# NYXFLOWER/GripNet

Measured on NVIDIA B200. Metric: GripNet fwd+bwd edges/sec per epoch (pose-0 shape), higher is better.
Workload: dtype f32

## Files before the change

gripnet_b200/csrc/gemm.cu:

```cuda
#include "common.cuh"

namespace gn {

constexpr int kBK = 16;
constexpr int kGemmThreads = 256;
constexpr int kTargetCtas = 148 * 2;
constexpr int kMaxSplits = 3 * 148;

struct GemmParams {
  int M, N, K;
  const float* A; int64_t lda;
  const float* B; int64_t ldb;
  float* C; int64_t ldc;
  int batch; int64_t sA, sB, sC;
  int batch_reduce;
  float alpha; int accumulate;
  const float* addend; int64_t ldd;
  const float* mask; int64_t ldm;
  const int64_t* a_rows;
  int kt;
  int iters;
  int splits;
  int iters_per_split;
  int vec_ok;
  float* ws;
};

struct GemmPlan {
  int cfg;
  int bm, bn, bk;
  int splits, iters_per_split, iters, kt;
  int batch_indep;
};

static GemmPlan make_plan(int M, int N, int K, int batch, int batch_reduce, int allow_split) {
  GemmPlan pl;
  if (M >= 1024) {
    if (N <= 16) { pl.cfg = 2; pl.bm = 128; pl.bn = 16; }
    else if (N <= 32) { pl.cfg = 1; pl.bm = 128; pl.bn = 32; }
    else { pl.cfg = 0; pl.bm = 64; pl.bn = 64; }
  } else if (M <= 32 || N <= 32 || int64_t(M) * N <= 4096 * 4) {
    pl.cfg = 3; pl.bm = 32; pl.bn = 32;
  } else {
    pl.cfg = 0; pl.bm = 64; pl.bn = 64;
  }
  pl.bk = kBK;
  if (pl.cfg == 3 && K >= 256) { pl.cfg = 4; pl.bk = 64; }
  pl.kt = int(ceil_div(K, pl.bk));
  pl.batch_indep = batch_reduce ? 1 : batch;
  pl.iters = (batch_reduce ? batch : 1) * pl.kt;
  const int64_t tiles = ceil_div(M, pl.bm) * ceil_div(N, pl.bn) * pl.batch_indep;
  int splits = 1;
  if (allow_split && pl.iters >= 4 && tiles < kTargetCtas) {
    int64_t want = (pl.bk >= 64 ? 3 * 148 : kTargetCtas) / tiles;
    int64_t cap = pl.bk >= 64 ? pl.iters : pl.iters / 2;
    splits = int(want < cap ? want : cap);
    if (splits > kMaxSplits) splits = kMaxSplits;
    if (splits < 1) splits = 1;
  }
  pl.iters_per_split = int(ceil_div(pl.iters > 0 ? pl.iters : 1, splits));
  pl.splits = int(ceil_div(pl.iters > 0 ? pl.iters : 1, pl.iters_per_split));
  return pl;
}

template <int TN>
__device__ __forceinline__ void epilogue_row(const GemmParams& p, float* C, int m, int n0, const float (&v)[TN]) {
  float r[TN];
#pragma unroll
  for (int j = 0; j < TN; ++j) r[j] = v[j] * p.alpha;
  float* crow = C + int64_t(m) * p.ldc + n0;
  if (TN == 4 && p.vec_ok && n0 + 3 < p.N) {
    if (p.accumulate) {
      const float4 c = *reinterpret_cast<const float4*>(crow);
      r[0] += c.x; r[1] += c.y; r[2] += c.z; r[3] += c.w;
    }
    if (p.addend) {
      const float4 a = *reinterpret_cast<const float4*>(p.addend + int64_t(m) * p.ldd + n0);
      r[0] += a.x; r[1] += a.y; r[2] += a.z; r[3] += a.w;
    }
    if (p.mask) {
      const float4 k = *reinterpret_cast<const float4*>(p.mask + int64_t(m) * p.ldm + n0);
      if (!(k.x > 0.f)) r[0] = 0.f;
      if (!(k.y > 0.f)) r[1] = 0.f;
      if (!(k.z > 0.f)) r[2] = 0.f;
      if (!(k.w > 0.f)) r[3] = 0.f;
    }
    *reinterpret_cast<float4*>(crow) = make_float4(r[0], r[1], r[2], r[3]);
    return;
  }
#pragma unroll
  for (int j = 0; j < TN; ++j) {
    const int n = n0 + j;
    if (n >= p.N) break;
    float x = r[j];
    if (p.accumulate) x += crow[j];
    if (p.addend) x += p.addend[int64_t(m) * p.ldd + n];
    if (p.mask && !(p.mask[int64_t(m) * p.ldm + n] > 0.f)) x = 0.f;
    crow[j] = x;
  }
}

template <bool TA, bool TB, int BM, int BN, int TM, int TN, int BK>
__global__ void __launch_bounds__(kGemmThreads) sgemm_kernel(const GemmParams p) {
  constexpr int NTX = BN / TN;
  static_assert((BM / TM) * NTX == kGemmThreads, "tile / micro-tile mismatch");
  __shared__ __align__(16) float As[BK][BM + 4];
  __shared__ __align__(16) float Bs[BK][BN + 4];
  const int tid = threadIdx.x;
  const int tx = tid % NTX, ty = tid / NTX;
  const int m0 = blockIdx.x * BM, n0 = blockIdx.y * BN;
  const int zb = blockIdx.z / p.splits;
  const int zs = blockIdx.z - zb * p.splits;

  const int it_begin = zs * p.iters_per_split;
  const int it_end = min(p.iters, it_begin + p.iters_per_split);

  float acc[TM][TN];
#pragma unroll
  for (int i = 0; i < TM; ++i)
#pragma unroll
    for (int j = 0; j < TN; ++j) acc[i][j] = 0.f;

  for (int it = it_begin; it < it_end; ++it) {
    int b, k0;
    if (p.batch_reduce) { b = it / p.kt; k0 = (it - b * p.kt) * BK; } else { b = zb; k0 = it * BK; }
    const float* A = p.A + int64_t(b) * p.sA;
    const float* B = p.B + int64_t(b) * p.sB;
#pragma unroll
    for (int i = 0; i < (BM * BK) / kGemmThreads; ++i) {
      const int e = tid + i * kGemmThreads;
      int m, k;
      if (!TA) { k = e % BK; m = e / BK; } else { m = e % BM; k = e / BM; }
      const int gm = m0 + m, gk = k0 + k;
      float v = 0.f;
      if (gm < p.M && gk < p.K) {
        if (!TA) {
          const int64_t r = p.a_rows ? p.a_rows[gm] : gm;
          v = __ldg(A + r * p.lda + gk);
        } else {
          const int64_t r = p.a_rows ? p.a_rows[gk] : gk;
          v = __ldg(A + r * p.lda + gm);
        }
      }
      As[k][m] = v;
    }
#pragma unroll
    for (int i = 0; i < (BN * BK) / kGemmThreads; ++i) {
      const int e = tid + i * kGemmThreads;
      int n, k;
      if (!TB) { n = e % BN; k = e / BN; } else { k = e % BK; n = e / BK; }
      const int gn_ = n0 + n, gk = k0 + k;
      float v = 0.f;
      if (gn_ < p.N && gk < p.K) v = !TB ? __ldg(B + int64_t(gk) * p.ldb + gn_) : __ldg(B + int64_t(gn_) * p.ldb + gk);
      Bs[k][n] = v;
    }
    __syncthreads();
#pragma unroll
    for (int k = 0; k < BK; ++k) {
      float a[TM], bb[TN];
#pragma unroll
      for (int i = 0; i < TM; ++i) a[i] = As[k][ty * TM + i];
#pragma unroll
      for (int j = 0; j < TN; ++j) bb[j] = Bs[k][tx * TN + j];
#pragma unroll
      for (int i = 0; i < TM; ++i)
#pragma unroll
        for (int j = 0; j < TN; ++j) acc[i][j] = fmaf(a[i], bb[j], acc[i][j]);
    }
    __syncthreads();
  }

  if (p.splits > 1) {
    float* W = p.ws + (int64_t(zb) * p.splits + zs) * p.M * p.N;
#pragma unroll
    for (int i = 0; i < TM; ++i) {
      const int m = m0 + ty * TM + i;
      if (m >= p.M) continue;
#pragma unroll
      for (int j = 0; j < TN; ++j) {
        const int n = n0 + tx * TN + j;
        if (n < p.N) W[int64_t(m) * p.N + n] = acc[i][j];
      }
    }
    return;
  }
  float* C = p.C + (p.batch_reduce ? 0 : int64_t(zb) * p.sC);
#pragma unroll
  for (int i = 0; i < TM; ++i) {
    const int m = m0 + ty * TM + i;
    if (m < p.M) epilogue_row<TN>(p, C, m, n0 + tx * TN, acc[i]);
  }
}

template <int LANES>
__global__ void __launch_bounds__(256) splitk_reduce_kernel(const GemmParams p, int batch_indep) {
  const int64_t t = int64_t(blockIdx.x) * blockDim.x + threadIdx.x;
  const int64_t idx = t / LANES;
  const int lane = int(t % LANES);
  const int64_t mn = int64_t(p.M) * p.N;
  if (idx >= mn * batch_indep) return;
  const int zb = int(idx / mn);
  const int64_t o = idx - int64_t(zb) * mn;
  const float* w = p.ws + int64_t(zb) * p.splits * mn + o;
  float s = 0.f;
  int z = lane;
  for (; z + 3 * LANES < p.splits; z += 4 * LANES) {
    const float a = __ldcg(w + int64_t(z) * mn), b = __ldcg(w + int64_t(z + LANES) * mn);
    const float c = __ldcg(w + int64_t(z + 2 * LANES) * mn), d = __ldcg(w + int64_t(z + 3 * LANES) * mn);
    s += a; s += b; s += c; s += d;
  }
  for (; z < p.splits; z += LANES) s += __ldcg(w + int64_t(z) * mn);
  if (LANES == 32) {
#pragma unroll
    for (int off = 16; off > 0; off >>= 1) s += __shfl_xor_sync(kFull, s, off);
    if (lane != 0) return;
  }
  const float v[1] = {s};
  epilogue_row<1>(p, p.C + (p.batch_reduce ? 0 : int64_t(zb) * p.sC), int(o / p.N), int(o % p.N), v);
}

template <bool TA, bool TB>
static int launch_cfg(const GemmPlan& pl, const GemmParams& p, dim3 grid, cudaStream_t st) {
  switch (pl.cfg) {
    case 0: GN_LAUNCH((sgemm_kernel<TA, TB, 64, 64, 4, 4, 16>), grid, kGemmThreads, 0, st, p); break;
    case 1: GN_LAUNCH((sgemm_kernel<TA, TB, 128, 32, 4, 4, 16>), grid, kGemmThreads, 0, st, p); break;
    case 2: GN_LAUNCH((sgemm_kernel<TA, TB, 128, 16, 2, 4, 16>), grid, kGemmThreads, 0, st, p); break;
    case 3: GN_LAUNCH((sgemm_kernel<TA, TB, 32, 32, 2, 2, 16>), grid, kGemmThreads, 0, st, p); break;
    default: GN_LAUNCH((sgemm_kernel<TA, TB, 32, 32, 2, 2, 64>), grid, kGemmThreads, 0, st, p); break;
  }
  return GN_OK;
}

}

using namespace gn;

extern "C" size_t gn_sgemm_workspace_bytes(int32_t M, int32_t N, int32_t K, int32_t batch, int batch_reduce) {
  if (M <= 0 || N <= 0 || K <= 0 || batch < 1) return 0;
  const GemmPlan pl = make_plan(M, N, K, batch, batch_reduce, 1);
  if (pl.splits <= 1) return 0;
  return size_t(pl.batch_indep) * pl.splits * M * N * sizeof(float);
}

extern "C" int gn_sgemm(int transA, int transB, int32_t M, int32_t N, int32_t K, const float* A, int64_t lda,
                        const float* B, int64_t ldb, float* C, int64_t ldc, int32_t batch, int64_t strideA,
                        int64_t strideB, int64_t strideC, int batch_reduce, float alpha, int accumulate,
                        const float* addend, int64_t ld_addend, const float* relu_mask, int64_t ld_mask,
                        const int64_t* a_rows, int32_t split_k, float* ws, size_t ws_bytes, void* stream) {
  if (M < 0 || N < 0 || K < 0 || batch < 1 || !C) return GN_ERR_ARG;
  if (M == 0 || N == 0) return GN_OK;
  if (K > 0 && (!A || !B)) return GN_ERR_ARG;
  cudaStream_t st = as_stream(stream);
  const GemmPlan pl = make_plan(M, N, K, batch, batch_reduce, split_k > 0 && ws != nullptr);
  GemmParams p;
  p.M = M; p.N = N; p.K = K;
  p.A = A; p.lda = lda; p.B = B; p.ldb = ldb; p.C = C; p.ldc = ldc;
  p.batch = batch; p.sA = strideA; p.sB = strideB; p.sC = strideC;
  p.batch_reduce = batch_reduce ? 1 : 0;
  p.alpha = alpha; p.accumulate = accumulate ? 1 : 0;
  p.addend = addend; p.ldd = ld_addend; p.mask = relu_mask; p.ldm = ld_mask;
  p.a_rows = a_rows;
  p.kt = pl.kt; p.iters = pl.iters; p.splits = pl.splits; p.iters_per_split = pl.iters_per_split;
  p.ws = ws;
  auto al16 = [](const void* q) { return (reinterpret_cast<uintptr_t>(q) & 15u) == 0; };
  p.vec_ok = al16(C) && ldc % 4 == 0 && (batch_reduce || batch == 1 || strideC % 4 == 0) &&
             (!addend || (al16(addend) && ld_addend % 4 == 0)) && (!relu_mask || (al16(relu_mask) && ld_mask % 4 == 0));
  if (pl.splits > 1 && ws_bytes < size_t(pl.batch_indep) * pl.splits * M * N * sizeof(float)) return GN_ERR_WORKSPACE;
  const int64_t gz = int64_t(pl.batch_indep) * pl.splits;
  dim3 grid((unsigned)ceil_div(M, pl.bm), (unsigned)ceil_div(N, pl.bn), (unsigned)gz);
  if (grid.y > 65535 || gz > 65535) return GN_ERR_RANGE;
  if (!transA && !transB) GN_CHECK((launch_cfg<false, false>(pl, p, grid, st)));
  else if (!transA && transB) GN_CHECK((launch_cfg<false, true>(pl, p, grid, st)));
  else if (transA && !transB) GN_CHECK((launch_cfg<true, false>(pl, p, grid, st)));
  else GN_CHECK((launch_cfg<true, true>(pl, p, grid, st)));
  if (pl.splits > 1) {
    const int64_t total = int64_t(M) * N * pl.batch_indep;
    if (pl.splits >= 16 && total <= 8192) {
      GN_LAUNCH(splitk_reduce_kernel<32>, (unsigned)ceil_div(total * 32, 256), 256, 0, st, p, pl.batch_indep);
    } else {
      GN_LAUNCH(splitk_reduce_kernel<1>, (unsigned)ceil_div(total, 256), 256, 0, st, p, pl.batch_indep);
    }
  }
  return GN_OK;
}
```

gripnet_b200/ops.py:

```python
import os
import weakref

import torch

from . import _lib, streams
from .graph import _ptr, _stream, _ws, require_cuda, validate_index

EPS = 1e-13


class M:
    __slots__ = ("t", "ptr", "ld", "n", "f")

    def __init__(self, t, col0=0, width=None):
        assert t.dim() == 2 and t.stride(1) == 1 and t.dtype == torch.float32
        self.t = t
        self.n = t.size(0)
        self.f = t.size(1) - col0 if width is None else width
        self.ld = t.stride(0) if t.size(0) > 1 else max(t.size(1), 1)
        self.ptr = t.data_ptr() + 4 * col0


def _as_rows(x, name):
    require_cuda(x, name)
    if x.dtype != torch.float32:
        raise RuntimeError(f"gripnet_b200: {name} must be float32")
    if x.dim() != 2:
        raise RuntimeError(f"gripnet_b200: {name} must be 2-D")
    if x.stride(1) != 1 or (x.size(0) > 1 and x.stride(0) < x.size(1)):
        x = x.contiguous()
    return x


def _new(n, f, like):
    return torch.empty((n, f), dtype=torch.float32, device=like.device)


class Slot:
    __slots__ = ("m", "full", "dctx", "halo")

    def __init__(self, n_local, f, like, dctx=None, block=None, halo=None):
        self.dctx, self.halo = dctx, halo
        if dctx is None:
            t = _new(n_local, f, like)
            self.m, self.full = M(t), M(t)
        elif halo is not None:
            buf = dctx.slot_buffer(halo.rows, f, like, uniform=False)
            self.full = M(buf)
            self.m = M(buf[:n_local])
        else:
            buf = dctx.slot_buffer(dctx.world * block, f, like)
            self.full = M(buf)
            self.m = M(buf[dctx.rank * block: dctx.rank * block + n_local])

    def gather(self):
        if self.dctx is not None:
            if self.halo is not None:
                self.dctx.halo_gather(self.full.t, self.halo)
            else:
                self.dctx.all_gather_slots(self.full.t)
        return self.full


def _reduce(dctx, t):
    if dctx is not None:
        dctx.reduce_param_grad_(t)
    return t


def spmm(csr, x, out, F, row_scale=None, bias=None, addend=None, relu=False):
    lib = _lib.load()
    partial = csr.partial(min(F, 128))
    _lib.check(lib.gn_spmm(csr.ref, x.ptr, x.ld, F, _ptr(row_scale), _ptr(bias),
                           addend.ptr if addend is not None else None, addend.ld if addend is not None else 0,
                           int(relu), out.ptr, out.ld, _ptr(partial), _stream()), "gn_spmm")


GEMM_PATH = os.environ.get("GRIPNET_B200_GEMM", "auto")
_TC_MIN_M = 4096


def _tc_eligible(ta, m, n, k, a_ptr, lda, c_ptr, ldc, batch, alpha, accumulate, addend, mask, a_rows):
    if GEMM_PATH == "ffma" or ta or batch != 1 or a_rows is not None or accumulate or alpha != 1.0:
        return False
    if GEMM_PATH != "tc" and (m < _TC_MIN_M or k < 16):
        return False
    if k % 4 or lda % 4 or ldc % 4 or a_ptr % 16 or c_ptr % 16 or k > 4096:
        return False
    for e in (addend, mask):
        if e is not None and (e.ld % 4 or e.ptr % 16):
            return False
    return True


def sgemm(ta, tb, m, n, k, a_ptr, lda, b_ptr, ldb, c_ptr, ldc, device, batch=1, sa=0, sb=0, sc=0, batch_reduce=False,
          alpha=1.0, accumulate=False, addend=None, mask=None, a_rows=None, split_k=True):
    lib = _lib.load()
    if m > 0 and n > 0 and k > 0 and _tc_eligible(ta, m, n, k, a_ptr, lda, c_ptr, ldc, batch, alpha, accumulate,
                                                  addend, mask, a_rows):
        nbytes = int(lib.gn_tc_gemm_workspace_bytes(m, n, k))
        if nbytes:
            img = _ws(nbytes, device)
            _lib.check(lib.gn_tc_gemm(int(tb), m, n, k, a_ptr, lda, b_ptr, ldb, c_ptr, ldc,
                                      addend.ptr if addend is not None else None,
                                      addend.ld if addend is not None else 0,
                                      mask.ptr if mask is not None else None, mask.ld if mask is not None else 0,
                                      _ptr(img), nbytes, _stream()), "gn_tc_gemm")
            return
    ws, ws_bytes = None, 0
    if split_k:
        ws_bytes = int(lib.gn_sgemm_workspace_bytes(m, n, k, batch, int(batch_reduce)))
        if ws_bytes:
            ws = torch.empty(ws_bytes // 4, dtype=torch.float32, device=device)
            streams.keep(ws)
    _lib.check(lib.gn_sgemm(int(ta), int(tb), m, n, k, a_ptr, lda, b_ptr, ldb, c_ptr, ldc, batch, sa, sb, sc,
                            int(batch_reduce), float(alpha), int(accumulate),
                            addend.ptr if addend is not None else None, addend.ld if addend is not None else 0,
                            mask.ptr if mask is not None else None, mask.ld if mask is not None else 0,
                            _ptr(a_rows), 1 if ws is not None else 0, _ptr(ws), ws_bytes, _stream()), "gn_sgemm")


def _rel_tc_ok(k, ldx, ldy, x_ptr, y_ptr):
    return GEMM_PATH != "ffma" and k % 4 == 0 and ldx % 4 == 0 and ldy % 4 == 0 and x_ptr % 16 == 0 and y_ptr % 16 == 0


def rel_transform(x, w, y, r, k, f, device, image=None):
    lib = _lib.load()
    n = x.n
    if n == 0:
        return
    if _rel_tc_ok(k, x.ld, y.ld, x.ptr, y.ptr):
        if image is not None:
            _lib.check(lib.gn_tc_gemm_rel_image(n, r, f, k, x.ptr, x.ld, _ptr(image), image.numel(), y.ptr, y.ld,
                                                _stream()), "gn_tc_gemm_rel_image")
            return
        nbytes = int(lib.gn_tc_gemm_rel_workspace_bytes(n, r, f, k))
        if nbytes:
            img = _ws(nbytes, device)
            _lib.check(lib.gn_tc_gemm_rel(n, r, f, k, x.ptr, x.ld, w.data_ptr(), y.ptr, y.ld, _ptr(img), nbytes,
                                          _stream()), "gn_tc_gemm_rel")
            return
    sgemm(False, False, n, f, k, x.ptr, x.ld, w.data_ptr(), f, y.ptr, y.ld, device, batch=r, sa=0, sb=k * f, sc=f)


def rel_weights(basis, att):
    nb, k, f = basis.shape
    r = att.size(0)
    bs, at = basis.contiguous(), att.contiguous()
    w = torch.empty((r, k, f), dtype=torch.float32, device=basis.device)
    sgemm(False, False, r, k * f, nb, at.data_ptr(), nb, bs.data_ptr(), k * f, w.data_ptr(), k * f, basis.device)
    return w


class RelPrologue:

    _pending = {}

    def __init__(self, layers, n_rows):
        lib = _lib.load()
        self.branch = streams.Branch(background=True)
        self.entries = []
        flat = [t for pair in layers for t in pair]
        with self.branch(*flat):
            for basis, att in layers:
                w = rel_weights(basis.detach(), att.detach())
                nb, k, f = basis.shape
                r = att.size(0)
                image = None
                nbytes = int(lib.gn_tc_gemm_rel_workspace_bytes(n_rows, r, f, k)) if GEMM_PATH != "ffma" and k % 4 == 0 else 0
                if nbytes and n_rows > 0:
                    image = _ws(nbytes, basis.device)
                    _lib.check(lib.gn_tc_rel_image(n_rows, r, f, k, w.data_ptr(), _ptr(image), nbytes, _stream()),
                               "gn_tc_rel_image")
                key = (basis.data_ptr(), att.data_ptr())
                entry = (self.branch, basis._version, att._version, int(n_rows), w, image)
                RelPrologue._pending.pop(key, None)
                RelPrologue._pending[key] = entry
                self.entries.append(key)
        while len(RelPrologue._pending) > 16:
            RelPrologue._pending.pop(next(iter(RelPrologue._pending)))

    @staticmethod
    def take(basis, att, n_rows):
        e = RelPrologue._pending.pop((basis.data_ptr(), att.data_ptr()), None)
        if e is None:
            return None
        branch, vb, va, rows, w, image = e
        branch.join()
        if vb != basis._version or va != att._version:
            return None
        return w, (image if rows == int(n_rows) else None)


_TC_TN_MIN_ROWS = 1 << 15


def weight_grad(a, b, out, device, c_inner=0, c_stride=0, force_tc=False):
    lib = _lib.load()
    n, mo, no = a.n, a.f, b.f
    ok = GEMM_PATH != "ffma" and n > 0 and mo % 4 == 0 and no % 4 == 0 and a.ld % 4 == 0 and b.ld % 4 == 0 and \
        a.ptr % 16 == 0 and b.ptr % 16 == 0 and (force_tc or GEMM_PATH == "tc" or n >= _TC_TN_MIN_ROWS)
    if not ok:
        return False
    nbytes = int(lib.gn_tc_tn_workspace_bytes(n, mo, no))
    if not nbytes:
        return False
    ws = _ws(nbytes, device)
    _lib.check(lib.gn_tc_tn(a.ptr, a.ld, b.ptr, b.ld, n, mo, no, out.data_ptr(), no, int(c_inner), int(c_stride),
                            _ptr(ws), nbytes, _stream()), "gn_tc_tn")
    return True


def map2d(op, src, dst):
    _lib.check(_lib.load().gn_map2d(op, src.ptr, src.ld, dst.ptr, dst.ld, src.n, src.f, _stream()), "gn_map2d")


def relu_bwd(g, y, dst):
    _lib.check(_lib.load().gn_relu_bwd(g.ptr, g.ld, y.ptr, y.ld, dst.ptr, dst.ld, g.n, g.f, _stream()), "gn_relu_bwd")


def colsum(x, out):
    lib = _lib.load()
    ws = _ws(lib.gn_colsum_workspace_bytes(x.n, x.f), out.device)
    _lib.check(lib.gn_colsum(x.ptr, x.ld, x.n, x.f, _ptr(out), _ptr(ws), ws.numel(), _stream()), "gn_colsum")


class GcnStack(torch.autograd.Function):
    @staticmethod
    def forward(ctx, x0, graph, relu_flags, catout, *params):
        n_layers = len(relu_flags)
        weights = [params[2 * l] for l in range(n_layers)]
        biases = [params[2 * l + 1] for l in range(n_layers)]
        x0 = _as_rows(x0, "x")
        if x0.size(0) != graph.n_src:
            raise RuntimeError(f"x has {x0.size(0)} rows but the graph has {graph.n_src} source nodes")
        if catout and graph.n_src != graph.n_dst:
            raise RuntimeError("if_catout needs a square graph")
        dims = [x0.size(1)] + [w.size(1) for w in weights]
        for l, w in enumerate(weights):
            require_cuda(w, "weight", torch.float32)
            if w.size(0) != dims[l]:
                raise RuntimeError(f"layer {l}: weight expects {w.size(0)} input features, got {dims[l]}")
        dev = x0.device
        dctx = getattr(graph, "ctx", None)
        b_src = graph.b_src if dctx is not None else None
        outs = []
        br = streams.Branch()
        if catout:
            buf = _new(graph.n_dst, sum(dims), x0)
            offs = [sum(dims[:i]) for i in range(len(dims))]
            h0 = M(buf, offs[0], dims[0])
            outs.append(h0)
        else:
            buf = None
            outs.append(M(x0))
        for l in range(n_layers):
            w = weights[l].contiguous()
            k, f = dims[l], dims[l + 1]
            y = Slot(graph.n_src, f, x0, dctx, b_src, getattr(graph, "fwd_halo", None))
            xin = M(x0) if l == 0 else outs[l]
            sgemm(False, False, graph.n_src, f, k, xin.ptr, xin.ld, w.data_ptr(), f, y.m.ptr, y.m.ld, dev)
            if l == 0 and catout:
                with br(x0):
                    map2d(_lib.EW_COPY, M(x0), h0)
            if catout:
                hl = M(buf, offs[l + 1], f)
            else:
                hl = M(_new(graph.n_dst, f, x0))
            b = biases[l].contiguous() if biases[l] is not None else None
            spmm(graph.fwd, y.gather(), hl, f, bias=b, relu=relu_flags[l])
            outs.append(hl)
        br.join()
        ctx.graph, ctx.relu_flags, ctx.catout, ctx.dims = graph, relu_flags, catout, dims
        ctx.has_bias = [b is not None for b in biases]
        ctx.param_refs = [None if p is None else weakref.ref(p) for p in params]
        ws = [w.contiguous() for w in weights]
        acts = [buf] if catout else [o.t for o in outs]
        ctx.n_acts = len(acts)
        ctx.save_for_backward(*acts, *ws)
        return buf if catout else outs[-1].t

    @staticmethod
    def backward(ctx, grad_out):
        graph, relu_flags, catout, dims = ctx.graph, ctx.relu_flags, ctx.catout, ctx.dims
        n_layers = len(relu_flags)
        saved = ctx.saved_tensors
        acts, weights = saved[: ctx.n_acts], saved[ctx.n_acts:]
        if catout:
            offs0 = [sum(dims[:i]) for i in range(len(dims))]
            outs = [M(acts[0], offs0[i], dims[i]) for i in range(len(dims))]
        else:
            outs = [M(a) for a in acts]
        g = _as_rows(grad_out, "grad")
        dev = g.device
        dctx = getattr(graph, "ctx", None)
        b_dst = graph.b_dst if dctx is not None else None
        bwd_halo = getattr(graph, "bwd_halo", None)
        if catout:
            offs = [sum(dims[:i]) for i in range(len(dims))]
            gs = [M(g, offs[i], dims[i]) for i in range(len(dims))]
            dh = gs[n_layers]
        else:
            gs = None
            dh = M(g)
        grads = [None] * (2 * n_layers)
        dz_slot = None
        dx0 = None
        br = streams.Branch(enabled=dctx is None or dctx.defer_grad_reduce, background=True)
        br_b = streams.Branch(enabled=dctx is None or dctx.defer_grad_reduce, background=True)
        for l in range(n_layers, 0, -1):
            f, k = dims[l], dims[l - 1]
            h_l, h_prev = outs[l], outs[l - 1]
            if dz_slot is not None:
                dz = dz_slot
            elif relu_flags[l - 1]:
                dz = Slot(graph.n_dst, f, g, dctx, b_dst, bwd_halo)
                relu_bwd(dh, h_l, dz.m)
            elif dctx is not None:
                dz = Slot(graph.n_dst, f, g, dctx, b_dst, bwd_halo)
                map2d(_lib.EW_COPY, dh, dz.m)
            else:
                dz = Slot.__new__(Slot)
                dz.m, dz.full, dz.dctx = dh, dh, None
            if ctx.has_bias[l - 1] and ctx.needs_input_grad[4 + 2 * (l - 1) + 1]:
                db = torch.empty(f, dtype=torch.float32, device=dev)
                with br_b(dz.m.t):
                    colsum(dz.m, db)
                grads[2 * (l - 1) + 1] = _reduce(dctx, db)
            dy = M(_new(graph.n_src, f, g))
            spmm(graph.bwd, dz.gather(), dy, f)
            if ctx.needs_input_grad[4 + 2 * (l - 1)]:
                dw = torch.empty((k, f), dtype=torch.float32, device=dev)
                with br(dy.t, h_prev.t):
                    if not weight_grad(h_prev, dy, dw, dev):
                        sgemm(True, False, k, f, graph.n_src, h_prev.ptr, h_prev.ld, dy.ptr, dy.ld, dw.data_ptr(),
                              f, dev)
                grads[2 * (l - 1)] = _reduce(dctx, dw)
            need_prev = (l > 1) or ctx.needs_input_grad[0]
            dz_slot = None
            if need_prev:
                w = weights[l - 1]
                addend = gs[l - 1] if catout else None
                mask = h_prev if (l > 1 and relu_flags[l - 2]) else None
                dprev = Slot(graph.n_src, k, g, dctx if mask is not None else None, b_dst, bwd_halo)
                sgemm(False, True, graph.n_src, k, f, dy.ptr, dy.ld, w.data_ptr(), f, dprev.m.ptr, dprev.m.ld, dev,
                      addend=addend, mask=mask)
                dh = dprev.m
                if mask is not None:
                    dz_slot = dprev
                if l == 1:
                    dx0 = dprev.m.t
        defer = _only_stored(ctx, dctx)
        br_b.join(deferrable=defer)
        br.join(deferrable=defer)
        return (dx0, None, None, None) + tuple(grads)


def _only_stored(ctx, dctx):
    if dctx is not None and not dctx.defer_grad_reduce:
        return False
    params = [None if r is None else r() for r in ctx.param_refs]
    return streams.grads_only_stored(params, ctx.needs_input_grad[4:])


class RgcnStack(torch.autograd.Function):
    @staticmethod
    def forward(ctx, x0, graph, relu_flags, catout, *params):
        n_layers = len(relu_flags)
        basis = [params[4 * l] for l in range(n_layers)]
        att = [params[4 * l + 1] for l in range(n_layers)]
        root = [params[4 * l + 2] for l in range(n_layers)]
        bias = [params[4 * l + 3] for l in range(n_layers)]
        x0 = _as_rows(x0, "x")
        n, r = graph.n_nodes, graph.n_rel
        if x0.size(0) != n:
            raise RuntimeError(f"x has {x0.size(0)} rows but the graph has {n} nodes")
        dims = [x0.size(1)] + [rt.size(1) for rt in root]
        dev = x0.device
        dctx = getattr(graph, "ctx", None)
        blk = graph.b if dctx is not None else None
        outs, ws_list = [], []
        br = streams.Branch()
        if catout:
            buf = _new(n, sum(dims), x0)
            offs = [sum(dims[:i]) for i in range(len(dims))]
            h0 = M(buf, offs[0], dims[0])
            with br(x0):
                map2d(_lib.EW_COPY, M(x0), h0)
            outs.append(h0)
        else:
            buf = None
            outs.append(M(x0))
        for l in range(n_layers):
            k, f = dims[l], dims[l + 1]
            nb = basis[l].size(0)
            if att[l].size(0) != r:
                raise RuntimeError("att rows must equal the number of relations of the graph")
            bs, at, rt = basis[l].contiguous(), att[l].contiguous(), root[l].contiguous()
            n_in = n if dctx is None else dctx.world * blk
            pre = RelPrologue.take(basis[l], att[l], n_in)
            w, image = pre if pre is not None else (rel_weights(bs, at), None)
            xin = M(x0) if l == 0 else outs[l]
            hl = M(buf, offs[l + 1], f) if catout else M(_new(n, f, x0))
            with br(xin.t, rt, hl.t):
                sgemm(False, False, n, f, k, xin.ptr, xin.ld, rt.data_ptr(), f, hl.ptr, hl.ld, dev)
            if dctx is not None:
                xs = Slot(n, k, x0, dctx, blk)
                map2d(_lib.EW_COPY, xin, xs.m)
                xall = xs.gather()
            else:
                xall = xin
            yfull = _new(xall.n, r * f, x0)
            rel_transform(xall, w, M(yfull), r, k, f, dev, image=image if xall.n == n_in else None)
            b = bias[l].contiguous() if bias[l] is not None else None
            br.join()
            spmm(graph.fwd, M(yfull.view(yfull.size(0) * r, f)), hl, f, row_scale=graph.inv_cnt, bias=b, addend=hl,
                 relu=relu_flags[l])
            outs.append(hl)
            ws_list.append((w, bs, at, rt))
        br.join()
        ctx.graph, ctx.relu_flags, ctx.catout, ctx.dims = graph, relu_flags, catout, dims
        ctx.has_bias = [b is not None for b in bias]
        ctx.param_refs = [None if p is None else weakref.ref(p) for p in params]
        acts = [buf] if catout else [o.t for o in outs]
        ctx.n_acts = len(acts)
        flat = [t for tup in ws_list for t in tup]
        ctx.save_for_backward(*acts, *flat)
        return buf if catout else outs[-1].t

    @staticmethod
    def backward(ctx, grad_out):
        graph, relu_flags, catout, dims = ctx.graph, ctx.relu_flags, ctx.catout, ctx.dims
        n_layers = len(relu_flags)
        n, r = graph.n_nodes, graph.n_rel
        saved = ctx.saved_tensors
        acts, flat = saved[: ctx.n_acts], saved[ctx.n_acts:]
        ws_list = [tuple(flat[4 * i: 4 * i + 4]) for i in range(n_layers)]
        if catout:
            offs0 = [sum(dims[:i]) for i in range(len(dims))]
            outs = [M(acts[0], offs0[i], dims[i]) for i in range(len(dims))]
        else:
            outs = [M(a) for a in acts]
        g = _as_rows(grad_out, "grad")
        dev = g.device
        dctx = getattr(graph, "ctx", None)
        blk = graph.b if dctx is not None else None
        if catout:
            offs = [sum(dims[:i]) for i in range(len(dims))]
            gs = [M(g, offs[i], dims[i]) for i in range(len(dims))]
            dh = gs[n_layers]
        else:
            gs = None
            dh = M(g)
        grads = [None] * (4 * n_layers)
        dz_slot = None
        dx0 = None
        br = streams.Branch(enabled=dctx is None or dctx.defer_grad_reduce, background=True)
        for l in range(n_layers, 0, -1):
            f, k = dims[l], dims[l - 1]
            w, bs, at, rt = ws_list[l - 1]
            nb = bs.size(0)
            h_l, h_prev = outs[l], outs[l - 1]
            if dz_slot is not None:
                dzs = dz_slot
            elif relu_flags[l - 1]:
                dzs = Slot(n, f, g, dctx, blk)
                relu_bwd(dh, h_l, dzs.m)
            elif dctx is not None:
                dzs = Slot(n, f, g, dctx, blk)
                map2d(_lib.EW_COPY, dh, dzs.m)
            else:
                dzs = Slot.__new__(Slot)
                dzs.m, dzs.full, dzs.dctx = dh, dh, None
            dz = dzs.m
            base = 4 + 4 * (l - 1)
            if ctx.has_bias[l - 1] and ctx.needs_input_grad[base + 3]:
                db = torch.empty(f, dtype=torch.float32, device=dev)
                with br(dz.t):
                    colsum(dz, db)
                grads[4 * (l - 1) + 3] = _reduce(dctx, db)
            dy = torch.empty((n * r, f), dtype=torch.float32, device=dev)
            spmm(graph.bwd, dzs.gather(), M(dy), f)
            if ctx.needs_input_grad[base + 2]:
                droot = torch.empty((k, f), dtype=torch.float32, device=dev)
                with br(dz.t, h_prev.t):
                    sgemm(True, False, k, f, n, h_prev.ptr, h_prev.ld, dz.ptr, dz.ld, droot.data_ptr(), f, dev)
                grads[4 * (l - 1) + 2] = _reduce(dctx, droot)
            if ctx.needs_input_grad[base] or ctx.needs_input_grad[base + 1]:
                dw = torch.empty((r, k, f), dtype=torch.float32, device=dev)
                datt = torch.empty((r, nb), dtype=torch.float32, device=dev) if ctx.needs_input_grad[base + 1] else None
                dbasis = torch.empty((nb, k, f), dtype=torch.float32, device=dev) if ctx.needs_input_grad[base] else None
                with br(dy, h_prev.t, dw, bs, at):
                    if not weight_grad(h_prev, M(dy.view(n, r * f)), dw, dev, c_inner=f, c_stride=k * f,
                                       force_tc=True):
                        sgemm(True, False, k, f, n, h_prev.ptr, h_prev.ld, dy.data_ptr(), r * f, dw.data_ptr(), f,
                              dev, batch=r, sa=0, sb=f, sc=k * f)
                    if datt is not None:
                        sgemm(False, True, r, nb, k * f, dw.data_ptr(), k * f, bs.data_ptr(), k * f, datt.data_ptr(),
                              nb, dev)
                    if dbasis is not None:
                        sgemm(True, False, nb, k * f, r, at.data_ptr(), nb, dw.data_ptr(), k * f, dbasis.data_ptr(),
                              k * f, dev)
                if datt is not None:
                    grads[4 * (l - 1) + 1] = _reduce(dctx, datt)
                if dbasis is not None:
                    grads[4 * (l - 1)] = _reduce(dctx, dbasis)
            need_prev = (l > 1) or ctx.needs_input_grad[0]
            dz_slot = None
            if need_prev:
                addend = gs[l - 1] if catout else None
                mask = h_prev if (l > 1 and relu_flags[l - 2]) else None
                dps = Slot(n, k, g, dctx if mask is not None else None, blk)
                dprev = dps.m
                sgemm(False, True, n, k, f, dz.ptr, dz.ld, rt.data_ptr(), f, dprev.ptr, dprev.ld, dev, addend=addend)
                sgemm(False, True, n, k, f, dy.data_ptr(), r * f, w.data_ptr(), f, dprev.ptr, dprev.ld, dev,
                      batch=r, sa=f, sb=k * f, sc=0, batch_reduce=True, accumulate=True, mask=mask)
                dh = dprev
                if mask is not None:
                    dz_slot = dps
                if l == 1:
                    dx0 = dprev.t
        br.join(deferrable=_only_stored(ctx, dctx))
        return (dx0, None, None, None) + tuple(grads)


def axpby(a, alpha, b, beta, dst):
    _lib.check(_lib.load().gn_axpby(a.ptr, a.ld, float(alpha), b.ptr if b is not None else None,
                                    b.ld if b is not None else 0, float(beta), dst.ptr, dst.ld, a.n, a.f,
                                    _stream()), "gn_axpby")


class Mean3(torch.autograd.Function):

    @staticmethod
    def forward(ctx, a, b, c):
        a, b, c = _as_rows(a, "a"), _as_rows(b, "b"), _as_rows(c, "c")
        if a.shape != b.shape or a.shape != c.shape:
            raise RuntimeError("mean3: the three inputs must have the same shape")
        out = _new(a.size(0), a.size(1), a)
        ma, mb, mc, mo = M(a), M(b), M(c), M(out)
        _lib.check(_lib.load().gn_mean3(ma.ptr, ma.ld, mb.ptr, mb.ld, mc.ptr, mc.ld, mo.ptr, mo.ld, ma.n, ma.f,
                                        _stream()), "gn_mean3")
        return out

    @staticmethod
    def backward(ctx, g):
        g = _as_rows(g, "grad")
        dg = _new(g.size(0), g.size(1), g)
        axpby(M(g), 1.0 / 3.0, None, 0.0, M(dg))
        return dg, dg, dg


def mean3(a, b, c):
    return Mean3.apply(a, b, c)


def abs_bwd(g, t, dst, scale):
    _lib.check(_lib.load().gn_abs_bwd(g.ptr, g.ld, t.ptr, t.ld, dst.ptr, dst.ld, g.n, g.f, float(scale),
                                      _stream()), "gn_abs_bwd")


class InterTail(torch.autograd.Function):
    @staticmethod
    def forward(ctx, h, target_feat, target_feat_down, mod, dctx=None):
        ctx.dctx = dctx
        h = _as_rows(h, "h")
        t = _as_rows(target_feat, "target_feat")
        n, f, ft = h.size(0), h.size(1), t.size(1)
        if t.size(0) != n:
            raise RuntimeError("target_feat rows must equal the number of target nodes")
        dev = h.device
        ctx.shapes = (n, f, ft)
        if mod == "cat":
            out = _new(n, f + ft, h)
            map2d(_lib.EW_COPY, M(h), M(out, 0, f))
            map2d(_lib.EW_ABS, M(t), M(out, f, ft))
            ctx.kind = 0
            ctx.save_for_backward(t)
            return out
        out = _new(n, f, h)
        if f == ft:
            map2d(_lib.EW_ABS, M(t), M(out))
            ctx.kind = 1
            ctx.save_for_backward(t)
        else:
            d = _as_rows(target_feat_down, "target_feat_down")
            u = _new(n, f, h)
            sgemm(False, False, n, f, ft, t.data_ptr(), t.stride(0), d.data_ptr(), d.stride(0), u.data_ptr(), f, dev)
            map2d(_lib.EW_RELU, M(u), M(out))
            ctx.kind = 2
            ctx.save_for_backward(t, d, u)
        axpby(M(h), 0.5, M(out), 0.5, M(out))
        return out

    @staticmethod
    def backward(ctx, grad):
        n, f, ft = ctx.shapes
        g = _as_rows(grad, "grad")
        dev = g.device
        if ctx.kind == 0:
            (t,) = ctx.saved_tensors
            dt = _new(n, ft, g)
            abs_bwd(M(g, f, ft), M(t), M(dt), 1.0)
            return g[:, :f], dt, None, None, None
        dh = _new(n, f, g)
        axpby(M(g), 0.5, None, 0.0, M(dh))
        if ctx.kind == 1:
            (t,) = ctx.saved_tensors
            dt = _new(n, ft, g)
            abs_bwd(M(g), M(t), M(dt), 0.5)
            return dh, dt, None, None, None
        t, d, u = ctx.saved_tensors
        du = _new(n, f, g)
        relu_bwd(M(dh), M(u), M(du))
        dt = _new(n, ft, g)
        sgemm(False, True, n, ft, f, du.data_ptr(), f, d.data_ptr(), d.stride(0), dt.data_ptr(), ft, dev)
        dd = torch.empty((ft, f), dtype=torch.float32, device=dev)
        sgemm(True, False, ft, f, n, t.data_ptr(), t.stride(0), du.data_ptr(), f, dd.data_ptr(), f, dev)
        return dh, dt, _reduce(ctx.dctx, dd), None, None


def _distmult_check(z, weight, edge_index, edge_type):
    z = _as_rows(z, "z")
    w = _as_rows(weight, "weight").contiguous()
    require_cuda(edge_index, "edge_index", torch.int64)
    require_cuda(edge_type, "edge_type", torch.int64)
    if edge_index.dim() != 2 or edge_index.size(0) != 2 or edge_type.numel() != edge_index.size(1):
        raise RuntimeError("edge_index must be [2,E] and edge_type [E]")
    if w.size(1) != z.size(1):
        raise RuntimeError("decoder weight width must equal the embedding width")
    validate_index(edge_index, z.size(0), "edge_index")
    validate_index(edge_type, w.size(0), "edge_type")
    return z, w, edge_index.contiguous(), edge_type.contiguous()


def _ldz(z):
    return z.stride(0) if z.size(0) > 1 else z.size(1)


def _distmult_fwd(z, w, ei, et, sigmoid):
    e = ei.size(1)
    out = torch.empty(e, dtype=torch.float32, device=z.device)
    _lib.check(_lib.load().gn_distmult_fwd(z.data_ptr(), _ldz(z), z.size(1), w.data_ptr(),
                                           _ptr(ei[0]) if e else None, _ptr(ei[1]) if e else None,
                                           _ptr(et) if e else None, e, int(sigmoid), _ptr(out), _stream()),
               "gn_distmult_fwd")
    return out


def _distmult_coef(g, out, sigmoid):
    e = out.numel()
    coef = torch.empty(max(e, 1), dtype=torch.float32, device=out.device)
    _lib.check(_lib.load().gn_distmult_coef(_ptr(g), _ptr(out), e, int(sigmoid), _ptr(coef), _stream()),
               "gn_distmult_coef")
    return coef


def _pair_walk(ps, coef, z):
    d = z.size(1)
    t = torch.empty((ps.csr.n_rows, d), dtype=torch.float32, device=z.device)
    part = ps.csr.partial(d)
    _lib.check(_lib.load().gn_distmult_bwd_pairs(ps.csr.ref, _ptr(ps.ent_other), _ptr(ps.ent_eid), _ptr(coef),
                                                 z.data_ptr(), _ldz(z), d, t.data_ptr(), _ptr(part), _stream()),
               "gn_distmult_bwd_pairs")
    return t


def _distmult_grads(t, t2, z, w, need_z, need_w):
    n, d, r = z.size(0), z.size(1), w.size(0)
    dz = torch.empty((n, d), dtype=torch.float32, device=z.device) if need_z else None
    dw = torch.empty_like(w) if need_w else None
    if need_z or need_w:
        lib = _lib.load()
        ws = _ws(lib.gn_distmult_grads_workspace_bytes(n, r, d), z.device)
        _lib.check(lib.gn_distmult_grads(t.data_ptr(), _ptr(t2), n, r, d, z.data_ptr(), _ldz(z), w.data_ptr(),
                                         _ptr(dz), d, _ptr(dw), _ptr(ws), ws.numel(), _stream()), "gn_distmult_grads")
    return dz, dw


def _check_versions(tensors, versions, what):
    for t, v in zip(tensors, versions):
        if t._version != v:
            raise RuntimeError(f"gripnet_b200: {what} was modified in place between forward and backward")


class DistMult(torch.autograd.Function):
    @staticmethod
    def forward(ctx, z, weight, edge_index, edge_type, sigmoid):
        from .graph import pair_struct
        z, w, ei, et = _distmult_check(z, weight, edge_index, edge_type)
        need = ctx.needs_input_grad[0] or ctx.needs_input_grad[1]
        br = streams.Branch()
        if need:
            with br(edge_index, edge_type):
                pair_struct(edge_index, edge_type, z.size(0), w.size(0))
        out = _distmult_fwd(z, w, ei, et, sigmoid)
        br.join()
        ctx.sigmoid = bool(sigmoid)
        ctx.key_tensors = (edge_index, edge_type)
        ctx.key_versions = (edge_index._version, edge_type._version)
        ctx.save_for_backward(z, w, out)
        return out

    @staticmethod
    def backward(ctx, grad):
        from .graph import pair_struct
        z, w, out = ctx.saved_tensors
        _check_versions(ctx.key_tensors, ctx.key_versions, "edge_index / edge_type")
        coef = _distmult_coef(grad.contiguous(), out, ctx.sigmoid)
        ps = pair_struct(ctx.key_tensors[0], ctx.key_tensors[1], z.size(0), w.size(0))
        t = _pair_walk(ps, coef, z)
        dz, dw = _distmult_grads(t, None, z, w, ctx.needs_input_grad[0], ctx.needs_input_grad[1])
        return dz, dw, None, None, None


class DistMultPair(torch.autograd.Function):

    @staticmethod
    def forward(ctx, z, weight, pos_index, neg_index, edge_type, sigmoid, rel_lo=0, n_rel_local=None,
                struct_branch=None):
        from .graph import pair_struct
        w_full = _as_rows(weight, "weight").contiguous()
        r_loc = w_full.size(0) if n_rel_local is None else int(n_rel_local)
        if rel_lo < 0 or rel_lo + r_loc > w_full.size(0):
            raise RuntimeError("relation slice out of range")
        w_loc = w_full[rel_lo: rel_lo + r_loc]
        z, w, pi, et = _distmult_check(z, w_loc, pos_index, edge_type)
        _, _, ni, _ = _distmult_check(z, w_loc, neg_index, edge_type)
        need = ctx.needs_input_grad[0] or ctx.needs_input_grad[1]
        br = streams.Branch()
        br_s = struct_branch if struct_branch is not None else streams.Branch(background=True)
        if need:
            with br_s(pos_index, neg_index, edge_type):
                pair_struct(neg_index, edge_type, z.size(0), r_loc)
                pair_struct(pos_index, edge_type, z.size(0), r_loc)
        with br(z, w, ni, et):
            neg = _distmult_fwd(z, w, ni, et, sigmoid)
        pos = _distmult_fwd(z, w, pi, et, sigmoid)
        br.join()
        if need and br_s._parent is None:
            ctx.struct_branch = br_s
        else:
            ctx.struct_branch = None
            br_s.join()
        ctx.sigmoid = bool(sigmoid)
        ctx.keys = (pos_index, neg_index, edge_type)
        ctx.key_versions = tuple(t._version for t in ctx.keys)
        ctx.rel = (int(rel_lo), r_loc, w_full.size(0))
        ctx.save_for_backward(z, w, pos, neg)
        return pos, neg

    @staticmethod
    def backward(ctx, g_pos, g_neg):
        from .graph import pair_struct
        z, w, pos, neg = ctx.saved_tensors
        pos_key, neg_key, et_key = ctx.keys
        _check_versions(ctx.keys, ctx.key_versions, "pos / neg edge_index or edge_type")
        rel_lo, r, r_full = ctx.rel
        n = z.size(0)
        if ctx.struct_branch is not None:
            ctx.struct_branch.join()
            ctx.struct_branch = None
        ps_p = pair_struct(pos_key, et_key, n, r)
        ps_n = pair_struct(neg_key, et_key, n, r)
        g_pos, g_neg = g_pos.contiguous(), g_neg.contiguous()
        br = streams.Branch(enabled=ps_p is not ps_n)
        with br(g_neg, neg, z):
            coef_n = _distmult_coef(g_neg, neg, ctx.sigmoid)
            t_n = _pair_walk(ps_n, coef_n, z)
        coef_p = _distmult_coef(g_pos, pos, ctx.sigmoid)
        t_p = _pair_walk(ps_p, coef_p, z)
        br.join()
        dz, dw = _distmult_grads(t_p, t_n, z, w, ctx.needs_input_grad[0], ctx.needs_input_grad[1])
        if dw is not None and r != r_full:
            dw_full = torch.empty((r_full, w.size(1)), dtype=torch.float32, device=w.device)
            _lib.check(_lib.load().gn_zero(dw_full.data_ptr(), dw_full.numel() * 4, _stream()), "gn_zero")
            map2d(_lib.EW_COPY, M(dw), M(dw_full[rel_lo: rel_lo + r]))
            dw = dw_full
        return dz, dw, None, None, None, None, None, None, None


class MultiClass(torch.autograd.Function):
    @staticmethod
    def forward(ctx, z, weight, node_list, softmax):
        lib = _lib.load()
        z = _as_rows(z, "z")
        w = _as_rows(weight, "weight").contiguous()
        require_cuda(node_list, "node_list", torch.int64)
        if w.size(0) != z.size(1):
            raise RuntimeError("decoder weight rows must equal the embedding width")
        validate_index(node_list, z.size(0), "node_list")
        idx = node_list.contiguous().view(-1)
        m, d, c = idx.numel(), z.size(1), w.size(1)
        dev = z.device
        logits = torch.empty((m, c), dtype=torch.float32, device=dev)
        sgemm(False, False, m, c, d, z.data_ptr(), z.stride(0) if z.size(0) > 1 else d, w.data_ptr(), c,
              logits.data_ptr(), c, dev, a_rows=idx)
        if softmax:
            out = torch.empty_like(logits)
            _lib.check(lib.gn_softmax_fwd(_ptr(logits), m, c, _ptr(out), _stream()), "gn_softmax_fwd")
        else:
            out = logits
        ctx.softmax = bool(softmax)
        ctx.key_tensor = node_list
        ctx.save_for_backward(z, w, out, idx)
        return out

    @staticmethod
    def backward(ctx, grad):
        from .graph import index_struct
        lib = _lib.load()
        z, w, out, idx = ctx.saved_tensors
        n, d, c, m = z.size(0), z.size(1), w.size(1), idx.numel()
        dev = z.device
        g = grad.contiguous()
        ldz = z.stride(0) if n > 1 else d
        if ctx.softmax:
            gl = torch.empty_like(g)
            _lib.check(lib.gn_softmax_bwd(_ptr(out), _ptr(g), m, c, _ptr(gl), _stream()), "gn_softmax_bwd")
        else:
            gl = g
        dz = dw = None
        if ctx.needs_input_grad[1]:
            dw = torch.empty((d, c), dtype=torch.float32, device=dev)
            sgemm(True, False, d, c, m, z.data_ptr(), ldz, gl.data_ptr(), c, dw.data_ptr(), c, dev, a_rows=idx)
        if ctx.needs_input_grad[0]:
            grows = torch.empty((max(m, 1), d), dtype=torch.float32, device=dev)
            sgemm(False, True, m, d, c, gl.data_ptr(), c, w.data_ptr(), c, grows.data_ptr(), d, dev)
            st = index_struct(ctx.key_tensor, n)
            dz = torch.empty((n, d), dtype=torch.float32, device=dev)
            spmm(st.csr, M(grows), M(dz), d)
        return dz, dw, None, None


class LinkPredLoss(torch.autograd.Function):
    @staticmethod
    def forward(ctx, pos, neg):
        lib = _lib.load()
        pos = require_cuda(pos, "pos_score", torch.float32).contiguous()
        neg = require_cuda(neg, "neg_score", torch.float32).contiguous()
        dev = pos.device
        loss = torch.empty(1, dtype=torch.float32, device=dev)
        n = max(pos.numel(), neg.numel())
        ws = _ws(lib.gn_loss_workspace_bytes(n), dev)
        _lib.check(lib.gn_lp_loss_fwd(_ptr(pos), pos.numel(), _ptr(neg), neg.numel(), EPS, _ptr(loss), _ptr(ws),
                                      ws.numel(), _stream()), "gn_lp_loss_fwd")
        ctx.save_for_backward(pos, neg)
        return loss.view(())

    @staticmethod
    def backward(ctx, grad):
        lib = _lib.load()
        pos, neg = ctx.saved_tensors
        g = grad.contiguous().view(1)
        gp, gn_ = torch.empty_like(pos), torch.empty_like(neg)
        _lib.check(lib.gn_lp_loss_bwd(_ptr(pos), pos.numel(), _ptr(neg), neg.numel(), EPS, _ptr(g), _ptr(gp),
                                      _ptr(gn_), _stream()), "gn_lp_loss_bwd")
        return gp, gn_


class NodeClassLoss(torch.autograd.Function):
    @staticmethod
    def forward(ctx, score, labels):
        lib = _lib.load()
        score = _as_rows(score, "score").contiguous()
        labels = require_cuda(labels, "labels", torch.int64).contiguous()
        if labels.numel() != score.size(0):
            raise RuntimeError("labels must have one entry per score row")
        validate_index(labels, score.size(1), "labels")
        dev = score.device
        loss = torch.empty(1, dtype=torch.float32, device=dev)
        ws = _ws(lib.gn_loss_workspace_bytes(score.size(0)), dev)
        _lib.check(lib.gn_nc_loss_fwd(_ptr(score), score.size(0), score.size(1), _ptr(labels), EPS, _ptr(loss),
                                      _ptr(ws), ws.numel(), _stream()), "gn_nc_loss_fwd")
        ctx.save_for_backward(score, labels)
        return loss.view(())

    @staticmethod
    def backward(ctx, grad):
        lib = _lib.load()
        score, labels = ctx.saved_tensors
        g = grad.contiguous().view(1)
        gs = torch.empty_like(score)
        _lib.check(lib.gn_nc_loss_bwd(_ptr(score), score.size(0), score.size(1), _ptr(labels), EPS, _ptr(g),
                                      _ptr(gs), _stream()), "gn_nc_loss_bwd")
        return gs, None


class MatMul(torch.autograd.Function):
    @staticmethod
    def forward(ctx, x, w):
        x = _as_rows(x, "x")
        w = _as_rows(w, "w").contiguous()
        out = _new(x.size(0), w.size(1), x)
        sgemm(False, False, x.size(0), w.size(1), x.size(1), x.data_ptr(), M(x).ld, w.data_ptr(), w.size(1),
              out.data_ptr(), w.size(1), x.device)
        ctx.save_for_backward(x, w)
        return out

    @staticmethod
    def backward(ctx, grad):
        x, w = ctx.saved_tensors
        g = _as_rows(grad, "grad")
        dx = dw = None
        if ctx.needs_input_grad[0]:
            dx = _new(x.size(0), x.size(1), x)
            sgemm(False, True, x.size(0), x.size(1), w.size(1), g.data_ptr(), M(g).ld, w.data_ptr(), w.size(1),
                  dx.data_ptr(), x.size(1), x.device)
        if ctx.needs_input_grad[1]:
            dw = _new(w.size(0), w.size(1), x)
            sgemm(True, False, w.size(0), w.size(1), x.size(0), x.data_ptr(), M(x).ld, g.data_ptr(), M(g).ld,
                  dw.data_ptr(), w.size(1), x.device)
        return dx, dw


def matmul(x, w):
    return MatMul.apply(x, w)
```

Baseline: 11.73 billion.

## Add narrow-GEMM kernel for small K and N and route skinny shapes to it

Adds a specialized SGEMM path for non-transposed A with K and N at most 64. The kernel stages all of B in shared memory once per CTA, and each thread computes four output columns of one row, looping over rows grid-stride. The tensor-core path is also skipped for such small shapes so they reach this FFMA kernel, which aims to cut tiling, split-K and tensor-core setup overhead on the skinny GEMMs that dominate GripNet layers. A probe script for timing these shapes is added alongside.

```diff
diff --git a/gripnet_b200/csrc/gemm.cu b/gripnet_b200/csrc/gemm.cu
--- a/gripnet_b200/csrc/gemm.cu
+++ b/gripnet_b200/csrc/gemm.cu
@@ -6,6 +6,9 @@
 constexpr int kGemmThreads = 256;
 constexpr int kTargetCtas = 148 * 2;
 constexpr int kMaxSplits = 3 * 148;
+constexpr int kNarrowMax = 64;
+constexpr int kNarrowThreads = 256;
+constexpr int kNarrowMaxCtas = 148 * 4;
 
 struct GemmParams {
   int M, N, K;
@@ -23,6 +26,7 @@
   int splits;
   int iters_per_split;
   int vec_ok;
+  int a_vec;
   float* ws;
 };
 
@@ -31,10 +35,21 @@
   int bm, bn, bk;
   int splits, iters_per_split, iters, kt;
   int batch_indep;
+  int smem;
 };
 
-static GemmPlan make_plan(int M, int N, int K, int batch, int batch_reduce, int allow_split) {
+
+static GemmPlan make_plan(int transA, int M, int N, int K, int batch, int batch_reduce, int allow_split) {
   GemmPlan pl;
+  pl.smem = 0;
+  if (!transA && batch == 1 && K > 16 && N <= kNarrowMax && K <= kNarrowMax) {
+    pl.cfg = 5; pl.bn = int(ceil_div(N, 4));
+    const int64_t spread = ceil_div(M, 148);
+    pl.bm = int(spread < kNarrowThreads / pl.bn ? spread : kNarrowThreads / pl.bn);
+    pl.bk = K; pl.kt = 1; pl.iters = 1; pl.splits = 1; pl.iters_per_split = 1; pl.batch_indep = 1;
+    pl.smem = int(K * pl.bn * 4 * sizeof(float));
+    return pl;
+  }
   if (M >= 1024) {
     if (N <= 16) { pl.cfg = 2; pl.bm = 128; pl.bn = 16; }
     else if (N <= 32) { pl.cfg = 1; pl.bm = 128; pl.bn = 32; }
@@ -219,6 +234,50 @@
   epilogue_row<1>(p, p.C + (p.batch_reduce ? 0 : int64_t(zb) * p.sC), int(o / p.N), int(o % p.N), v);
 }
 
+__device__ __forceinline__ void narrow_step(float4& acc, float x, const float4 t) {
+  acc.x = fmaf(x, t.x, acc.x); acc.y = fmaf(x, t.y, acc.y);
+  acc.z = fmaf(x, t.z, acc.z); acc.w = fmaf(x, t.w, acc.w);
+}
+
+__global__ void __launch_bounds__(kNarrowThreads, 2) narrow_kernel(const GemmParams p, int transB, int bm) {
+  extern __shared__ float4 bs4[];
+  float* Bs = reinterpret_cast<float*>(bs4);
+  const int nq = (p.N + 3) >> 2, np = nq * 4;
+  const int K = p.K;
+  for (int e = threadIdx.x; e < K * np; e += blockDim.x) {
+    const int k = e / np, n = e - k * np;
+    Bs[e] = n >= p.N ? 0.f : __ldg(transB ? p.B + int64_t(n) * p.ldb + k : p.B + int64_t(k) * p.ldb + n);
+  }
+  __syncthreads();
+
+  const int q = threadIdx.x % nq, r = threadIdx.x / nq;
+  if (r >= bm) return;
+  const float4* w = bs4 + q;
+  for (int64_t m = int64_t(blockIdx.x) * bm + r; m < p.M; m += int64_t(gridDim.x) * bm) {
+    const float* a = p.A + (p.a_rows ? p.a_rows[m] : m) * p.lda;
+    float4 acc = make_float4(0.f, 0.f, 0.f, 0.f);
+    if (p.a_vec) {
+      float4 x[kNarrowMax / 4];
+#pragma unroll
+      for (int i = 0; i < kNarrowMax / 4; ++i)
+        if (4 * i < K) x[i] = __ldg(reinterpret_cast<const float4*>(a) + i);
+#pragma unroll
+      for (int i = 0; i < kNarrowMax / 4; ++i) {
+        if (4 * i < K) {
+          narrow_step(acc, x[i].x, w[(4 * i) * nq]);
+          narrow_step(acc, x[i].y, w[(4 * i + 1) * nq]);
+          narrow_step(acc, x[i].z, w[(4 * i + 2) * nq]);
+          narrow_step(acc, x[i].w, w[(4 * i + 3) * nq]);
+        }
+      }
+    } else {
+      for (int k = 0; k < K; ++k) narrow_step(acc, __ldg(a + k), w[k * nq]);
+    }
+    const float v[4] = {acc.x, acc.y, acc.z, acc.w};
+    epilogue_row<4>(p, p.C, int(m), 4 * q, v);
+  }
+}
+
 template <bool TA, bool TB>
 static int launch_cfg(const GemmPlan& pl, const GemmParams& p, dim3 grid, cudaStream_t st) {
   switch (pl.cfg) {
@@ -237,7 +296,7 @@
 
 extern "C" size_t gn_sgemm_workspace_bytes(int32_t M, int32_t N, int32_t K, int32_t batch, int batch_reduce) {
   if (M <= 0 || N <= 0 || K <= 0 || batch < 1) return 0;
-  const GemmPlan pl = make_plan(M, N, K, batch, batch_reduce, 1);
+  const GemmPlan pl = make_plan(1, M, N, K, batch, batch_reduce, 1);
   if (pl.splits <= 1) return 0;
   return size_t(pl.batch_indep) * pl.splits * M * N * sizeof(float);
 }
@@ -251,7 +310,7 @@
   if (M == 0 || N == 0) return GN_OK;
   if (K > 0 && (!A || !B)) return GN_ERR_ARG;
   cudaStream_t st = as_stream(stream);
-  const GemmPlan pl = make_plan(M, N, K, batch, batch_reduce, split_k > 0 && ws != nullptr);
+  const GemmPlan pl = make_plan(transA, M, N, K, batch, batch_reduce, split_k > 0 && ws != nullptr);
   GemmParams p;
   p.M = M; p.N = N; p.K = K;
   p.A = A; p.lda = lda; p.B = B; p.ldb = ldb; p.C = C; p.ldc = ldc;
@@ -265,6 +324,14 @@
   auto al16 = [](const void* q) { return (reinterpret_cast<uintptr_t>(q) & 15u) == 0; };
   p.vec_ok = al16(C) && ldc % 4 == 0 && (batch_reduce || batch == 1 || strideC % 4 == 0) &&
              (!addend || (al16(addend) && ld_addend % 4 == 0)) && (!relu_mask || (al16(relu_mask) && ld_mask % 4 == 0));
+  if (pl.cfg == 5) {
+    p.a_vec = al16(A) && lda % 4 == 0 && K % 4 == 0;
+    const int64_t ctas = ceil_div(M, pl.bm);
+    GN_LAUNCH(narrow_kernel, (unsigned)(ctas < kNarrowMaxCtas ? ctas : kNarrowMaxCtas), kNarrowThreads, pl.smem, st, p,
+              transB ? 1 : 0, pl.bm);
+    return GN_OK;
+  }
+  p.a_vec = 0;
   if (pl.splits > 1 && ws_bytes < size_t(pl.batch_indep) * pl.splits * M * N * sizeof(float)) return GN_ERR_WORKSPACE;
   const int64_t gz = int64_t(pl.batch_indep) * pl.splits;
   dim3 grid((unsigned)ceil_div(M, pl.bm), (unsigned)ceil_div(N, pl.bn), (unsigned)gz);
diff --git a/gripnet_b200/ops.py b/gripnet_b200/ops.py
--- a/gripnet_b200/ops.py
+++ b/gripnet_b200/ops.py
@@ -78,12 +78,17 @@
 
 GEMM_PATH = os.environ.get("GRIPNET_B200_GEMM", "auto")
 _TC_MIN_M = 4096
+_NARROW_MAX_MKN = 1 << 25
+
+
+def _narrow_wins(m, n, k):
+    return k <= 64 and n <= 64 and m * k * n < _NARROW_MAX_MKN
 
 
 def _tc_eligible(ta, m, n, k, a_ptr, lda, c_ptr, ldc, batch, alpha, accumulate, addend, mask, a_rows):
     if GEMM_PATH == "ffma" or ta or batch != 1 or a_rows is not None or accumulate or alpha != 1.0:
         return False
-    if GEMM_PATH != "tc" and (m < _TC_MIN_M or k < 16):
+    if GEMM_PATH != "tc" and (m < _TC_MIN_M or k < 16 or _narrow_wins(m, n, k)):
         return False
     if k % 4 or lda % 4 or ldc % 4 or a_ptr % 16 or c_ptr % 16 or k > 4096:
         return False
diff --git a/profiles/narrow_gemm_probe.py b/profiles/narrow_gemm_probe.py
--- /dev/null
+++ b/profiles/narrow_gemm_probe.py
@@ -0,0 +1,108 @@
+#!/usr/bin/env python
+import argparse
+import json
+import os
+import sys
+
+ROOT = os.path.dirname(os.path.dirname(os.path.abspath(__file__)))
+sys.path.insert(0, ROOT)
+import torch
+
+SWEEP_M = [645, 19_081, 65_536, 262_144, 1 << 20]
+SWEEP_KN = [(32, 16), (16, 16), (16, 32), (64, 16), (16, 64), (48, 32), (32, 48), (64, 64)]
+CHAIN = [
+    ("gg1 X.W", 0, 0, 19_081, 16, 32, 1, 0),
+    ("gg2 X.W", 0, 0, 19_081, 16, 16, 1, 0),
+    ("gd X.W", 0, 0, 19_081, 16, 64, 1, 0),
+    ("rgcn root dX", 0, 1, 645, 48, 32, 1, 0),
+    ("rgcn rel dX (R=16)", 0, 1, 645, 48, 32, 16, 1),
+    ("gd dX", 0, 1, 19_081, 64, 16, 1, 0),
+    ("gg2 dX", 0, 1, 19_081, 16, 16, 1, 0),
+    ("gg1 dX", 0, 1, 19_081, 32, 16, 1, 0),
+    ("gg1 dW", 1, 0, 32, 16, 19_081, 1, 0),
+    ("gg2 dW", 1, 0, 16, 16, 19_081, 1, 0),
+]
+
+
+def main():
+    ap = argparse.ArgumentParser()
+    ap.add_argument("--tag", default="")
+    ap.add_argument("--quick", action="store_true", help="chain shapes only")
+    args = ap.parse_args()
+    from gripnet_b200 import _lib, ops
+    lib = _lib.load()
+    dev = torch.device("cuda:0")
+    flush = torch.empty(256 << 20, dtype=torch.uint8, device=dev)
+
+    def timeit(fn):
+        for _ in range(3):
+            fn()
+        torch.cuda.synchronize()
+        g = torch.cuda.CUDAGraph()
+        with torch.cuda.graph(g):
+            for _ in range(20):
+                fn()
+        g.replay()
+        torch.cuda.synchronize()
+        e0, e1 = torch.cuda.Event(enable_timing=True), torch.cuda.Event(enable_timing=True)
+        e0.record()
+        for _ in range(10):
+            g.replay()
+        e1.record()
+        torch.cuda.synchronize()
+        warm = e0.elapsed_time(e1) * 1e3 / 200
+        ts = []
+        for _ in range(15):
+            flush.zero_()
+            e0.record(); fn(); e1.record()
+            torch.cuda.synchronize()
+            ts.append(e0.elapsed_time(e1) * 1e3)
+        return round(warm, 2), round(sorted(ts)[len(ts) // 2], 2)
+
+    def run(name, ta, tb, m, n, k, batch, br):
+        a_rows, a_cols = (k, m) if ta else (m, k * batch)
+        a = torch.randn(a_rows, a_cols, device=dev)
+        b = torch.randn(batch, *((n, k) if tb else (k, n)), device=dev)
+        c = torch.zeros(m, n, device=dev)
+        lda, ldb = a_cols, (k if tb else n)
+        sa, sb = (k if br else 0), (n * k if br else 0)
+        ws_bytes = int(lib.gn_sgemm_workspace_bytes(m, n, k, batch, br))
+        ws = torch.empty(max(ws_bytes // 4, 1), device=dev)
+        rec = {"tag": args.tag, "name": name, "ta": ta, "tb": tb, "M": m, "N": n, "K": k, "batch": batch}
+
+        def sg():
+            _lib.check(lib.gn_sgemm(ta, tb, m, n, k, a.data_ptr(), lda, b.data_ptr(), ldb, c.data_ptr(), n, batch,
+                                    sa, sb, 0, br, 1.0, 0, None, 0, None, 0, None, 1 if ws_bytes else 0,
+                                    ws.data_ptr() if ws_bytes else None, ws_bytes,
+                                    torch.cuda.current_stream().cuda_stream), "gn_sgemm")
+        rec["sgemm_warm_us"], rec["sgemm_cold_us"] = timeit(sg)
+        ref = (a.double().view(m, batch, k).transpose(0, 1) @ (b.double().transpose(1, 2) if tb else b.double())).sum(0) \
+            if not ta else a.double().t() @ b.double()[0]
+        rec["sgemm_rel_err"] = float((c.double() - ref).abs().max() / ref.abs().max())
+        if not ta and batch == 1:
+            nbytes = int(lib.gn_tc_gemm_workspace_bytes(m, n, k)) if k % 4 == 0 else 0
+            if nbytes:
+                img = torch.empty(nbytes, dtype=torch.uint8, device=dev)
+
+                def tc():
+                    _lib.check(lib.gn_tc_gemm(tb, m, n, k, a.data_ptr(), lda, b.data_ptr(), ldb, c.data_ptr(), n,
+                                              None, 0, None, 0, img.data_ptr(), nbytes,
+                                              torch.cuda.current_stream().cuda_stream), "gn_tc_gemm")
+                rec["tc_warm_us"], rec["tc_cold_us"] = timeit(tc)
+
+            def auto():
+                ops.sgemm(False, bool(tb), m, n, k, a.data_ptr(), lda, b.data_ptr(), ldb, c.data_ptr(), n, dev)
+            rec["auto_warm_us"], rec["auto_cold_us"] = timeit(auto)
+        print(json.dumps(rec), flush=True)
+
+    for row in CHAIN:
+        run(*row)
+    if args.quick:
+        return
+    for m in SWEEP_M:
+        for k, n in SWEEP_KN:
+            run("sweep", 0, 0, m, n, k, 1, 0)
+
+
+if __name__ == "__main__":
+    main()
```

After: 12.75 billion, median of 6. 8.7% higher.
